# zyhbili/Dual-Space-NeRF

Measured on AMD Instinct MI355X. Metric: rendered rays/sec (64 samples/ray), 512x512 frame, higher is better.
Workload: dtype split-f16x3 (3 x v_mfma_f32_32x32x16_f16 on hi/lo fp16 operand halves, f32 accumulate: f32-equivalent accuracy - parity bars of the tests: 1e-4 absolute on RGB / acc / weights against the reference; sigma 1e-4 absolute where |sigma| <= 100 and 4e-6 RELATIVE to max|sigma| above (this checkpoint: |sig

## Files before the change

dual-space-nerf_amd/csrc/dsn_common.h:

```cpp
#pragma once
#include <hip/hip_runtime.h>
#include <stddef.h>
#include <stdint.h>

#define DSN_WAVE 64
#define DSN_NUM_PARAMS_INTERNAL 33

struct DsnFaceRec {
    float m0[3];
    float d00;
    float v10[3];
    float d01;
    float v20[3];
    float d11;
    float n[3];
    float inv;
};

#ifndef DSN_LIGHT_RECORD_FLOATS
#define DSN_LIGHT_RECORD_FLOATS 12
#endif
struct DsnLightEdit {
    float has_light, light_shift[3], has_rot, rot[4] , rot_center[2], pad;
};
static_assert(sizeof(DsnLightEdit) == 4 * DSN_LIGHT_RECORD_FLOATS, "DsnLightEdit is one light record");
__device__ __forceinline__ void dsn_light_edit(const DsnLightEdit& e, float (&xw)[3]) {
    if (e.has_rot != 0.0f) {
        const float ax = xw[0] - e.rot_center[0], ay = xw[1] - e.rot_center[1];
        const float nx = (ax * e.rot[0] + ay * e.rot[2]) + e.rot_center[0];
        const float ny = (ax * e.rot[1] + ay * e.rot[3]) + e.rot_center[1];
        xw[0] = nx; xw[1] = ny;
    }
    if (e.has_light != 0.0f) { xw[0] += e.light_shift[0]; xw[1] += e.light_shift[1]; xw[2] += e.light_shift[2]; }
}

struct DsnFrameState {
    float pose_feat[16];
    float code[8];
    DsnLightEdit light;
    float pad[28];
    float bias0[256];
};
static_assert(offsetof(DsnFrameState, bias0) == 256 && sizeof(DsnFrameState) == 1280, "DsnFrameState layout");

__host__ __device__ inline size_t dsn_align256(size_t x) { return (x + 255) & ~(size_t)255; }
#include "dsn_nn.h"

struct DsnSceneView {
    int V, F;
    float* canon;
    int32_t* faces;
    float* xyz;
    float4* cent_world;
    float4* cent_canon;
    DsnFaceRec* face_world;
    DsnFaceRec* face_canon;
    DsnFrameState* frame;
    DsnNNView nn_world;
    DsnNNView nn_canon;
};

__host__ __device__ inline DsnSceneView dsn_scene_view(void* base, int V, int F) {
    DsnSceneView s;
    char* p = (char*)base;
    s.V = V; s.F = F;
    p += 256;
    s.frame = (DsnFrameState*)p;    p += dsn_align256(sizeof(DsnFrameState));
    s.canon = (float*)p;            p += dsn_align256(sizeof(float) * 3 * (size_t)V);
    s.faces = (int32_t*)p;          p += dsn_align256(sizeof(int32_t) * 3 * (size_t)F);
    s.xyz = (float*)p;              p += dsn_align256(sizeof(float) * 3 * (size_t)V);
    s.cent_world = (float4*)p;      p += dsn_align256(sizeof(float4) * (size_t)F);
    s.cent_canon = (float4*)p;      p += dsn_align256(sizeof(float4) * (size_t)F);
    s.face_world = (DsnFaceRec*)p;  p += dsn_align256(sizeof(DsnFaceRec) * (size_t)F);
    s.face_canon = (DsnFaceRec*)p;  p += dsn_align256(sizeof(DsnFaceRec) * (size_t)F);
    s.nn_world = dsn_nn_view(p, F);
    s.nn_canon = dsn_nn_view(p, F);
    return s;
}
__host__ __device__ inline size_t dsn_pose_state_size() { return 256 + dsn_align256(sizeof(DsnFrameState)); }
__host__ __device__ inline size_t dsn_scene_size(int V, int F) {
    return 256 + 2 * dsn_align256(sizeof(float) * 3 * (size_t)V) + dsn_align256(sizeof(int32_t) * 3 * (size_t)F) +
           2 * dsn_align256(sizeof(float4) * (size_t)F) + 2 * dsn_align256(sizeof(DsnFaceRec) * (size_t)F) +
           dsn_align256(sizeof(DsnFrameState)) + 2 * dsn_nn_bytes(F);
}

__device__ __forceinline__ float dsn_sum3(float a, float b, float c) { return (a + b) + c; }
__device__ __forceinline__ float dsn_dot3(const float* a, const float* b) {
    return dsn_sum3(a[0] * b[0], a[1] * b[1], a[2] * b[2]);
}
__device__ __forceinline__ float dsn_norm3(const float* a) {
    return sqrtf(fmaf(a[2], a[2], fmaf(a[1], a[1], a[0] * a[0])));
}
__device__ __forceinline__ void dsn_cross3(const float* a, const float* b, float* o) {
    o[0] = fmaf(a[1], b[2], -(a[2] * b[1]));
    o[1] = fmaf(a[2], b[0], -(a[0] * b[2]));
    o[2] = fmaf(a[0], b[1], -(a[1] * b[0]));
}
__device__ __forceinline__ float dsn_div(float a, float b) { return __fdiv_rn(a, b); }

__device__ __forceinline__ void dsn_sincos(float x, float& s, float& c) {
    const float kf = rintf(x * 0.636619772367581343f);
    float r = fmaf(kf, -1.57079637050628662109375f, x);
    r = fmaf(kf, 4.37113900018624283e-8f, r);
    const float z = r * r;
    float ps = fmaf(z, -1.9515295891e-4f, 8.3321608736e-3f);
    ps = fmaf(z, ps, -1.6666654611e-1f);
    const float sr = fmaf(r * z, ps, r);
    float pc = fmaf(z, 2.443315711809948e-5f, -1.388731625493765e-3f);
    pc = fmaf(z, pc, 4.166664568298827e-2f);
    const float cr = fmaf(z * z, pc, fmaf(z, -0.5f, 1.0f));
    const int q = (int)kf;
    const float a = (q & 1) ? cr : sr;
    const float b = (q & 1) ? sr : cr;
    s = (q & 2) ? -a : a;
    c = ((q + 1) & 2) ? -b : b;
}
// ... 122 lines not shown
```

dual-space-nerf_amd/csrc/dsn_field16.hip:

```cpp
#include "dsn_common.h"
#include "dsn_kernels.h"

typedef float f32x16 __attribute__((ext_vector_type(16)));
typedef _Float16 half8 __attribute__((ext_vector_type(8)));
#define MFMA16(a, b, c) __builtin_amdgcn_mfma_f32_32x32x16_f16((a), (b), (c), 0, 0, 0)

#if !defined(DSN_EXPERIMENTS) && (defined(F16_ABL) || defined(F16_SABL) || defined(F16_TIMING) || defined(F16_TRAIN_ABL))
#error "F16_ABL / F16_SABL / F16_TIMING are experiment switches (wrong results / debug counters): build with -DDSN_EXPERIMENTS"
#endif
#ifndef F16_SINCOS_OCML
#define F16_SINCOS_OCML 0
#endif
#ifndef F16_FENCE
#define F16_FENCE 0
#endif
#ifndef F16_SGB
#define F16_SGB 1
#endif
#ifndef F16_SGB_VALU
#define F16_SGB_VALU 2
#endif
#ifndef F16_SGB_DS
#define F16_SGB_DS 1
#endif
#ifndef F16_MIX
#define F16_MIX 1
#endif
#ifndef F16_PIPE_LATE
#define F16_PIPE_LATE 1
#endif
#ifndef F16_ABL
#define F16_ABL 0
#endif
#ifndef F16_NEXT_POINT
#define F16_NEXT_POINT 1
#endif
#ifndef F16_DMA_SPREAD
#define F16_DMA_SPREAD 1
#endif
#ifndef F16_BIAS_AHEAD
#define F16_BIAS_AHEAD 1
#endif
#ifndef F16_TIMING
#define F16_TIMING 0
#endif
#ifndef F16_PREFETCH
#define F16_PREFETCH 1
#endif

#define F16_THREADS 256
#if defined(DSN_EXPERIMENTS) && defined(F16_TRAIN_ABL) && (F16_TRAIN_ABL & 32)
#define F16_ST_M(m) (1024 * (m))
#else
#define F16_ST_M(m) (32 * (m))
#endif
#define F16_CHUNK 8
#define F16_RING_SLOTS (2 * F16_CHUNK)
#define F16_NCHUNK (DSN_STREAM_BLOCKS / F16_CHUNK)
#define F16_RANGE 65000.0f
#define F16_RANGE_SCALED 32768.0f
#define F16_GSCALE 0.015625f
#define F16_GUNSCALE 64.0f

#if F16_TIMING
__device__ unsigned long long g_f16_timing[16];
#define F16_STAMP(i) do { if (MODE == F16_FWD) { asm volatile("s_waitcnt vmcnt(0) lgkmcnt(0)" ::: "memory"); tstamp[i] = __builtin_readcyclecounter(); rstamp[i] = wall_clock64(); } } while (0)
extern "C" __attribute__((visibility("default"))) int dsn_debug_timing(unsigned long long* out16, int reset) {
    if (out16 && hipMemcpyFromSymbol(out16, HIP_SYMBOL(g_f16_timing), sizeof(unsigned long long) * 16) != hipSuccess) return 1;
    if (reset) { unsigned long long z[16] = {0}; if (hipMemcpyToSymbol(HIP_SYMBOL(g_f16_timing), z, sizeof(z)) != hipSuccess) return 1; }
    return 0;
}
#else
#define F16_STAMP(i) do { } while (0)
#endif
struct W16 {
    const char* g;
    char* ring;
    unsigned ring_off;
    int wave;
    int nchunk = F16_NCHUNK;
    bool spread = F16_DMA_SPREAD != 0;
    half8 h0, l0, h1, l1;
};

#ifndef F16_POS_OFFS
#define F16_POS_OFFS 0
#endif
__device__ __forceinline__ void w16_stage(const W16& w, int c) {
    const char* src = w.g + (size_t)c * 32768;
    const unsigned dst = w.ring_off + (c & 1) * 32768 + w.wave * 8192 + 4096;
#if F16_POS_OFFS
// ... 124 lines not shown
#endif
            __builtin_amdgcn_sched_group_barrier(0x002, F16_SGB_VALU, 0);
        }
        __builtin_amdgcn_sched_barrier(0);
#endif
#if F16_FENCE
        __builtin_amdgcn_sched_barrier(0);
#endif
    }
}

__device__ __forceinline__ f32x16 rows16(const float* __restrict__ v, int m, int half) {
    f32x16 o;
#pragma unroll
    for (int q = 0; q < 4; ++q) {
        const float4 t = *reinterpret_cast<const float4*>(v + 32 * m + 8 * q + 4 * half);
        o[4 * q + 0] = t.x; o[4 * q + 1] = t.y; o[4 * q + 2] = t.z; o[4 * q + 3] = t.w;
    }
    return o;
}
__device__ __forceinline__ f32x16 zero16() {
    f32x16 z;
#pragma unroll
    for (int r = 0; r < 16; ++r) z[r] = 0.0f;
    return z;
}
template <bool SCALED>
__device__ __forceinline__ void split16(const f32x16& v, half8 (&h)[2], half8 (&l)[2]) {
#pragma unroll
    for (int r = 0; r < 16; ++r) {
        const _Float16 hi = (_Float16)v[r];
        const float res = fmaf((float)hi, -1.0f, v[r]);
        h[r >> 3][r & 7] = hi;
        l[r >> 3][r & 7] = SCALED ? (_Float16)(res * DSN_LO_SCALE) : (_Float16)res;
    }
}
#define F16_FWD_SCALE 64.0f
#define F16_FWD_INV 0.015625f
__device__ __forceinline__ f32x16 unscale16(const f32x16& m, const f32x16& c) {
    f32x16 v;
#pragma unroll
    for (int r = 0; r < 16; ++r) v[r] = (m[r] + c[r]) * F16_FWD_INV;
    return v;
}
__device__ __forceinline__ f32x16 fold16(const f32x16& m, const f32x16& c) {
    f32x16 v;
#pragma unroll
    for (int r = 0; r < 16; ++r) v[r] = fmaf(c[r], DSN_LO_INV, m[r]);
    return v;
}
__device__ __forceinline__ uint32_t dsn_push_sign(uint32_t word, float v) {
    return __builtin_amdgcn_alignbit(word, __float_as_uint(v), 31);
}
__device__ __forceinline__ uint32_t dsn_active_word(uint32_t signs) { return ~signs & 0xffffu; }
#ifndef F16_KEEP_ASM
#define F16_KEEP_ASM 1
#endif
__device__ __forceinline__ float dsn_keep_active(float v, uint32_t word, int r) {
#if F16_KEEP_ASM
    uint32_t m;
    asm("v_bfe_i32 %0, %1, %2, 1" : "=v"(m) : "v"(word), "s"(15 - r));
    return __uint_as_float(__float_as_uint(v) & m);
#else
    return __uint_as_float(__float_as_uint(v) & (uint32_t)__builtin_amdgcn_sbfe((int)word, 15 - r, 1));
#endif
}
__device__ __forceinline__ uint32_t relu_bits16(f32x16& a) {
    uint32_t s = 0;
#pragma unroll
    for (int r = 0; r < 16; ++r) {
        s = dsn_push_sign(s, a[r]);
        a[r] = fmaxf(a[r], 0.0f);
    }
    return dsn_active_word(s);
}
__device__ __forceinline__ void mask16(f32x16& a, uint32_t m) {
#pragma unroll
    for (int r = 0; r < 16; ++r) a[r] = dsn_keep_active(a[r], m, r);
}

__device__ __forceinline__ void track16(float& ovf, const f32x16& v) {
#pragma unroll
    for (int r = 0; r < 16; r += 2) asm("v_max3_f32 %0, %0, |%1|, |%2|" : "+v"(ovf) : "v"(v[r]), "v"(v[r + 1]));
}
__device__ __forceinline__ float dsn_nan_flag() { return __uint_as_float(0x7fc00000u); }

#if defined(DSN_EXPERIMENTS) && defined(F16_TRAIN_ABL) && (F16_TRAIN_ABL & 256)
__device__ __forceinline__ void store16_lines_emul(float* st, const float (&o)[16]) {
    const int lane = threadIdx.x & 63;
    const unsigned long long me = (unsigned long long)(uintptr_t)st;
#pragma unroll
    for (int j = 0; j < 4; ++j) {
        const int src = 8 * j + (lane >> 3);
        const unsigned lo = __shfl((unsigned)me, src), hi = __shfl((unsigned)(me >> 32), src);
        float* pj = reinterpret_cast<float*>((uintptr_t)(((unsigned long long)hi << 32) | lo));
        if (pj) *reinterpret_cast<float4*>(pj + 4 * (lane & 7)) = make_float4(o[4 * j], o[4 * j + 1], o[4 * j + 2], o[4 * j + 3]);
    }
}
#endif
template <bool FWD, bool ST = false, bool HEAD = false>
__device__ __forceinline__ void epi_slice(const f32x16& pM, const f32x16& pC, int kb, uint32_t mword, uint32_t& bits,
                                          half8 (&yh)[2], half8 (&yl)[2], float& ovf, float* st = nullptr, float stscale = 1.0f,
                                          const float* wd = nullptr, float* sg = nullptr) {
#if F16_ABL & 16
    {
        asm volatile("" : : "a"(pM[2 * kb]), "a"(pM[2 * kb + 1]), "a"(pC[2 * kb]), "a"(pC[2 * kb + 1]));
        if (kb == 0) { yh[0] = yh[1]; yl[0] = yl[1]; }
        return;
    }
#endif
    float vv[2];
#pragma unroll
    for (int e = 0; e < 2; ++e) {
        const int r = 2 * kb + e;
#if F16_ABL & 32
        asm volatile("" : : "v"(pC[r]));
        float v = FWD ? pM[r] * F16_FWD_INV : pM[r];
#else
        float v = FWD ? (pM[r] + pC[r]) * F16_FWD_INV : fmaf(pC[r], DSN_LO_INV, pM[r]);
#endif
        if (FWD) {
            bits = dsn_push_sign(bits, v);
            v = fmaxf(v, 0.0f);
        } else {
            v = dsn_keep_active(v, mword, r);
        }
        vv[e] = v;
        if (HEAD) *sg = fmaf(wd[8 * (r >> 2) + (r & 3)], v, *sg);
#if !F16_MIX
        const _Float16 hi = (_Float16)v;
        const float res = fmaf((float)hi, -1.0f, v);
        yh[r >> 3][r & 7] = hi;
        yl[r >> 3][r & 7] = FWD ? (_Float16)res : (_Float16)(res * DSN_LO_SCALE);
#endif
    }
#if F16_MIX
    {
        const int r = 2 * kb;
        uint32_t H, L;
        asm("v_cvt_pk_f16_f32 %0, %1, %2" : "=v"(H) : "v"(vv[0]), "v"(vv[1]));
        if (FWD) {
            asm("v_fma_mixlo_f16 %0, %1, -1.0, %2 op_sel_hi:[1,0,0]" : "=v"(L) : "v"(H), "v"(vv[0]));
            asm("v_fma_mixhi_f16 %0, %1, -1.0, %2 op_sel:[1,0,0] op_sel_hi:[1,0,0]" : "+v"(L) : "v"(H), "v"(vv[1]));
        } else {
            const float k = -DSN_LO_SCALE;
            const float s0 = vv[0] * DSN_LO_SCALE, s1 = vv[1] * DSN_LO_SCALE;
            asm("v_fma_mixlo_f16 %0, %1, %2, %3 op_sel_hi:[1,0,0]" : "=v"(L) : "v"(H), "s"(k), "v"(s0));
            asm("v_fma_mixhi_f16 %0, %1, %2, %3 op_sel:[1,0,0] op_sel_hi:[1,0,0]" : "+v"(L) : "v"(H), "s"(k), "v"(s1));
        }
        typedef uint32_t u32x4 __attribute__((ext_vector_type(4)));
        u32x4 th = __builtin_bit_cast(u32x4, yh[r >> 3]), tl = __builtin_bit_cast(u32x4, yl[r >> 3]);
        th[(r & 7) >> 1] = H;
        tl[(r & 7) >> 1] = L;
        yh[r >> 3] = __builtin_bit_cast(half8, th);
        yl[r >> 3] = __builtin_bit_cast(half8, tl);
    }
#endif
    if (FWD) asm("v_max3_f32 %0, %0, %1, %2" : "+v"(ovf) : "v"(vv[0]), "v"(vv[1]));
    else asm("v_max3_f32 %0, %0, |%1|, |%2|" : "+v"(ovf) : "v"(vv[0]), "v"(vv[1]));
#if defined(DSN_EXPERIMENTS) && defined(F16_TRAIN_ABL) && (F16_TRAIN_ABL & 256)
    if (ST && kb == 7) {
        float o[16];
#pragma unroll
        for (int r = 0; r < 16; ++r) {
            float v = FWD ? (pM[r] + pC[r]) * F16_FWD_INV : fmaf(pC[r], DSN_LO_INV, pM[r]);
            v = FWD ? fmaxf(v, 0.0f) : dsn_keep_active(v, mword, r);
// ... 1494 lines not shown
    for (int m = 0; m < 4; ++m) {
        f32x16 acc = rows16(packed + OFF_BLT1, m, half);
#pragma unroll
        for (int kb = 0; kb < 4; ++kb) {
            const float4* bp = reinterpret_cast<const float4*>(packed + OFF_LT1 + (m * 4 + kb) * DSN_BLK) + lane;
            const float4 c0 = bp[0], c1 = bp[64], c2 = bp[128], c3 = bp[192];
            acc = DSN_MFMA(c0.x, h1[kb][0], acc);  acc = DSN_MFMA(c0.y, h1[kb][1], acc);
            acc = DSN_MFMA(c0.z, h1[kb][2], acc);  acc = DSN_MFMA(c0.w, h1[kb][3], acc);
            acc = DSN_MFMA(c1.x, h1[kb][4], acc);  acc = DSN_MFMA(c1.y, h1[kb][5], acc);
            acc = DSN_MFMA(c1.z, h1[kb][6], acc);  acc = DSN_MFMA(c1.w, h1[kb][7], acc);
            acc = DSN_MFMA(c2.x, h1[kb][8], acc);  acc = DSN_MFMA(c2.y, h1[kb][9], acc);
            acc = DSN_MFMA(c2.z, h1[kb][10], acc); acc = DSN_MFMA(c2.w, h1[kb][11], acc);
            acc = DSN_MFMA(c3.x, h1[kb][12], acc); acc = DSN_MFMA(c3.y, h1[kb][13], acc);
            acc = DSN_MFMA(c3.z, h1[kb][14], acc); acc = DSN_MFMA(c3.w, h1[kb][15], acc);
        }
#pragma unroll
        for (int r = 0; r < 16; ++r) acc[r] = acc[r] > 0.0f ? acc[r] : 0.0f;
        h2[m] = acc;
    }
    float part = 0.0f;
#pragma unroll
    for (int m = 0; m < 4; ++m) {
        const f32x16 w = rows16(packed + OFF_WLT2, m, half);
#pragma unroll
        for (int r = 0; r < 16; ++r) part = fmaf(w[r], h2[m][r], part);
    }
    part += __shfl_xor(part, 32);
    return part + packed[OFF_SCAL + 4];
}

#define LIGHT32_THREADS 256
__global__ void __launch_bounds__(LIGHT32_THREADS, 1)
k_light(const float* __restrict__ packed, const DsnFrameState* __restrict__ fs, const float* __restrict__ n_w,
        const float* __restrict__ x_w_pts, const float* __restrict__ ray_o, const float* __restrict__ ray_d,
        const float* __restrict__ z_vals, const float* essence, int64_t N, int S,
        const int32_t* __restrict__ active_list, const int32_t* __restrict__ active_count,
        float* colour) {
    DSN_OWN_SIMD();
    const int lane = threadIdx.x & 63;
    const int wave = __builtin_amdgcn_readfirstlane(threadIdx.x >> 6);
    const int half = lane >> 5;
    const int64_t count = active_list ? (int64_t)(*active_count) : N;
    const int64_t slot0 = ((int64_t)blockIdx.x * 4 + wave) * 32;
    if (slot0 >= count) return;
    int64_t slot = slot0 + (lane & 31);
    const bool valid = slot < count;
    if (!valid) slot = count - 1;
    const int64_t pt = active_list ? (int64_t)active_list[slot] : slot;
    const int64_t ray = pt / S;

    float in9[10];
    in9[0] = n_w[3 * pt]; in9[1] = n_w[3 * pt + 1]; in9[2] = n_w[3 * pt + 2];
    float xw[3];
    const float d[3] = {ray_d[3 * ray], ray_d[3 * ray + 1], ray_d[3 * ray + 2]};
    if (x_w_pts) { xw[0] = x_w_pts[3 * pt]; xw[1] = x_w_pts[3 * pt + 1]; xw[2] = x_w_pts[3 * pt + 2]; }
    else {
        const float z = z_vals[pt];
        xw[0] = ray_o[3 * ray] + d[0] * z; xw[1] = ray_o[3 * ray + 1] + d[1] * z; xw[2] = ray_o[3 * ray + 2] + d[2] * z;
    }
    dsn_light_edit(fs->light, xw);
    in9[3] = xw[0]; in9[4] = xw[1]; in9[5] = xw[2];
    const float vn = dsn_norm3(d);
    in9[6] = dsn_div(d[0], vn); in9[7] = dsn_div(d[1], vn); in9[8] = dsn_div(d[2], vn);
    in9[9] = 0.0f;

    const float o = dsn_light_mlp32(packed, lane, in9);
    const float wgt = (o > 0.0f ? o : expm1f(o)) + 1.0f;
    if (valid && half == 0) {
        colour[3 * pt + 0] = wgt * essence[3 * pt + 0];
        colour[3 * pt + 1] = wgt * essence[3 * pt + 1];
        colour[3 * pt + 2] = wgt * essence[3 * pt + 2];
    }
}

void dsn_launch_light(const float* packed, const DsnFrameState* fs, const float* n_w, const float* x_w,
                      const float* ray_o, const float* ray_d, const float* z_vals, const float* essence, int64_t N,
                      int S, const int32_t* active_list, const int32_t* active_count, float* colour, hipStream_t st) {
    int64_t blocks = (N + 127) / 128;
    if (blocks == 0) return;
    hipLaunchKernelGGL(k_light, dim3((unsigned)blocks), dim3(LIGHT32_THREADS), 0, st, packed, fs, n_w, x_w, ray_o, ray_d,
                       z_vals, essence, N, S, active_list, active_count, colour);
}

__device__ __forceinline__ void light_block0(const char* blkp, int lane, const half8 (&xh)[2], const half8 (&xl)[2], f32x16& aM, f32x16& aC) {
    const half8 h0 = *reinterpret_cast<const half8*>(blkp + lane * 16);
    const half8 l0 = *reinterpret_cast<const half8*>(blkp + 1024 + lane * 16);
    aM = MFMA16(h0, xh[0], aM);
    aC = MFMA16(h0, xl[0], aC);
    aC = MFMA16(l0, xh[0], aC);
}
__device__ __forceinline__ void light_block(const char* __restrict__ blkp, int lane, const half8 (&xh)[2], const half8 (&xl)[2],
                                            f32x16& aM, f32x16& aC, bool second_step) {
    const half8 h0 = *reinterpret_cast<const half8*>(blkp + lane * 16);
    const half8 l0 = *reinterpret_cast<const half8*>(blkp + 1024 + lane * 16);
    aM = MFMA16(h0, xh[0], aM);
    aC = MFMA16(h0, xl[0], aC);
    aC = MFMA16(l0, xh[0], aC);
    if (second_step) {
        const half8 h1 = *reinterpret_cast<const half8*>(blkp + 2048 + lane * 16);
        const half8 l1 = *reinterpret_cast<const half8*>(blkp + 3072 + lane * 16);
        aM = MFMA16(h1, xh[1], aM);
        aC = MFMA16(h1, xl[1], aC);
        aC = MFMA16(l1, xh[1], aC);
    }
}

#define LIGHT_LDS_BYTES (4 * 2048 + 16 * 4096)
__device__ __forceinline__ void light16_stage_weights(const float* __restrict__ packed, char* s_w) {
    const char* g16 = reinterpret_cast<const char*>(packed + OFF16_BASE);
    const uint4* g0 = reinterpret_cast<const uint4*>(g16 + (size_t)(OFF_LT0 / DSN_BLK) * 4096);
    const uint4* g1 = reinterpret_cast<const uint4*>(g16 + (size_t)(OFF_LT1 / DSN_BLK) * 4096);
    uint4* d = reinterpret_cast<uint4*>(s_w);
    for (int i = threadIdx.x; i < 4 * 128; i += 256) d[i] = g0[(i >> 7) * 256 + (i & 127)];
    for (int i = threadIdx.x; i < 16 * 256; i += 256) d[4 * 128 + i] = g1[i];
    __syncthreads();
}
struct LightIn { float nw[3], o[3], d[3], z; };
__device__ __forceinline__ int64_t light16_tile_slot(int64_t t, int wave, int lane, int64_t ntiles, int64_t count, bool& ok) {
    int64_t sl = (t * 4 + wave) * 32 + (lane & 31);
    ok = t < ntiles && sl < count;
    if (!ok) sl = count - 1;
    return sl;
}
__device__ __forceinline__ void light16_fetch(int64_t p, int S, const float* __restrict__ n_w, const float* __restrict__ x_w_pts,
                                              const float* __restrict__ ray_o, const float* __restrict__ ray_d,
                                              const float* __restrict__ z_vals, LightIn& a) {
    const int64_t r = p / S;
    a.nw[0] = n_w[3 * p]; a.nw[1] = n_w[3 * p + 1]; a.nw[2] = n_w[3 * p + 2];
    a.d[0] = ray_d[3 * r]; a.d[1] = ray_d[3 * r + 1]; a.d[2] = ray_d[3 * r + 2];
    if (x_w_pts) { a.o[0] = x_w_pts[3 * p]; a.o[1] = x_w_pts[3 * p + 1]; a.o[2] = x_w_pts[3 * p + 2]; a.z = 0.0f; }
    else { a.o[0] = ray_o[3 * r]; a.o[1] = ray_o[3 * r + 1]; a.o[2] = ray_o[3 * r + 2]; a.z = z_vals[p]; }
}
__device__ __forceinline__ float light16_mlp(const float* __restrict__ packed, const char* s_w, int lane, const float (&in9)[10],
                                             bool valid, int64_t pt, float* __restrict__ tr_hl1, float* __restrict__ tr_hl2,
                                             bool& flagged) {
    const int half = lane >> 5;
    float ovf = packed[DSN_SPLIT_UNSAFE_LIGHT];
    half8 xh[2], xl[2];
    {
        f32x16 v = zero16();
#pragma unroll
        for (int j = 0; j < 5; ++j) v[j] = half ? in9[2 * j + 1] : in9[2 * j];
        track16(ovf, v);
        split16<true>(v, xh, xl);
    }
    half8 h1h[4][2], h1l[4][2];
#pragma unroll
    for (int m = 0; m < 4; ++m) {
        f32x16 aM = rows16(packed + OFF_BLT0, m, half), aC = zero16();
        light_block0(s_w + m * 2048, lane, xh, xl, aM, aC);
        f32x16 v = fold16(aM, aC);
#pragma unroll
        for (int r = 0; r < 16; ++r) v[r] = fmaxf(v[r], 0.0f);
        if (tr_hl1 && valid) store16(tr_hl1 + pt * 128 + 4 * half + 32 * m, v, 1.0f);
        track16(ovf, v);
        split16<true>(v, h1h[m], h1l[m]);
    }
    float part = 0.0f;
#pragma unroll
    for (int m = 0; m < 4; ++m) {
        f32x16 aM = rows16(packed + OFF_BLT1, m, half), aC = zero16();
#pragma unroll
        for (int kb = 0; kb < 4; ++kb)
            light_block(s_w + 4 * 2048 + (m * 4 + kb) * 4096, lane, h1h[kb], h1l[kb], aM, aC, true);
        f32x16 v = fold16(aM, aC);
        const f32x16 w2 = rows16(packed + OFF_WLT2, m, half);
#pragma unroll
        for (int r = 0; r < 16; ++r) { v[r] = fmaxf(v[r], 0.0f); part = fmaf(w2[r], v[r], part); }
        if (tr_hl2 && valid) store16(tr_hl2 + pt * 128 + 4 * half + 32 * m, v, 1.0f);
    }
    part += __shfl_xor(part, 32);
    float o = part + packed[OFF_SCAL + 4];
    flagged = !(fmaxf(ovf, __shfl_xor(ovf, 32)) < F16_RANGE_SCALED);
    if (__ballot(flagged)) {
        const float e = dsn_light_mlp32(packed, lane, in9);
        if (flagged) o = e;
    }
    return o;
}
__device__ __forceinline__ float light16_weight(float o) { return (o > 0.0f ? o : expm1f(o)) + 1.0f; }

template <bool FACTOR>
__global__ void __launch_bounds__(256, 1)
k_light16(const float* __restrict__ packed, const DsnFrameState* __restrict__ fs, const float* __restrict__ n_w,
          const float* __restrict__ x_w_pts, const float* __restrict__ ray_o, const float* __restrict__ ray_d,
          const float* __restrict__ z_vals, const float* essence, int64_t N, int S,
          const int32_t* __restrict__ active_list, const int32_t* __restrict__ active_count,
          float* colour, float* __restrict__ tr_hl1, float* __restrict__ tr_hl2, float* __restrict__ tr_pre,
          int32_t* __restrict__ range_count, float* __restrict__ factor) {
    __shared__ __attribute__((aligned(16))) char s_w[LIGHT_LDS_BYTES];
#ifndef F16_SHARE_SIMD
    DSN_OWN_SIMD();
#endif
    const int lane = threadIdx.x & 63;
    const int wave = __builtin_amdgcn_readfirstlane(threadIdx.x >> 6);
    const int half = lane >> 5;
    const int64_t count = active_list ? (int64_t)(*active_count) : N;
    const int64_t ntiles = (count + 127) / 128;
    if ((int64_t)blockIdx.x >= ntiles) return;
    light16_stage_weights(packed, s_w);
    auto tile_pt = [&](int64_t t, bool& ok) -> int64_t {
        const int64_t sl = light16_tile_slot(t, wave, lane, ntiles, count, ok);
        return active_list ? (int64_t)active_list[sl] : sl;
    };
    bool valid_c, valid_n, valid_nn;
    int64_t pt_c = tile_pt(blockIdx.x, valid_c);
    LightIn in_c, in_n;
    light16_fetch(pt_c, S, n_w, x_w_pts, ray_o, ray_d, z_vals, in_c);
    int64_t pt_n = tile_pt((int64_t)blockIdx.x + gridDim.x, valid_n);
  for (int64_t tile = blockIdx.x; tile < ntiles; tile += gridDim.x) {
    const int64_t slot0 = (tile * 4 + wave) * 32;
    const bool valid = valid_c;
    const int64_t pt = pt_c;
    const LightIn cur = in_c;
    light16_fetch(pt_n, S, n_w, x_w_pts, ray_o, ray_d, z_vals, in_n);
    const int64_t pt_nn = tile_pt(tile + 2 * (int64_t)gridDim.x, valid_nn);
    pt_c = pt_n; valid_c = valid_n; in_c = in_n;
    pt_n = pt_nn; valid_n = valid_nn;
    if (slot0 >= count) continue;
    const float ess[3] = {essence[3 * pt], essence[3 * pt + 1], essence[3 * pt + 2]};

    float in9[10];
    in9[0] = cur.nw[0]; in9[1] = cur.nw[1]; in9[2] = cur.nw[2];
    float xw[3];
    const float d[3] = {cur.d[0], cur.d[1], cur.d[2]};
    if (x_w_pts) { xw[0] = cur.o[0]; xw[1] = cur.o[1]; xw[2] = cur.o[2]; }
    else {
        const float z = cur.z;
        xw[0] = cur.o[0] + d[0] * z; xw[1] = cur.o[1] + d[1] * z; xw[2] = cur.o[2] + d[2] * z;
    }
    dsn_light_edit(fs->light, xw);
    in9[3] = xw[0]; in9[4] = xw[1]; in9[5] = xw[2];
    const float vn = dsn_norm3(d);
    in9[6] = dsn_div(d[0], vn); in9[7] = dsn_div(d[1], vn); in9[8] = dsn_div(d[2], vn);
    in9[9] = 0.0f;

    bool flagged;
    const float o = light16_mlp(packed, s_w, lane, in9, valid, pt, tr_hl1, tr_hl2, flagged);
    if (flagged && range_count && valid && half == 0) atomicAdd(range_count, 1);
    const float wgt = light16_weight(o);
    if (tr_pre && valid && half == 0) tr_pre[pt] = o;
    if (valid && half == 0) {
        colour[3 * pt + 0] = wgt * ess[0];
        colour[3 * pt + 1] = wgt * ess[1];
        colour[3 * pt + 2] = wgt * ess[2];
        if (FACTOR) factor[pt] = wgt;
    }
  }
}

void dsn_launch_light16(const float* packed, const DsnFrameState* fs, const float* n_w, const float* x_w,
                        const float* ray_o, const float* ray_d, const float* z_vals, const float* essence, int64_t N,
                        int S, const int32_t* active_list, const int32_t* active_count, float* colour, hipStream_t st,
                        float* tr_hl1, float* tr_hl2, float* tr_pre, int32_t* range_count, float* factor) {
    int64_t blocks = (N + 127) / 128;
    if (blocks == 0) return;
    const dim3 grid((unsigned)std::min<int64_t>(blocks, (int64_t)dsn_cu_count()));
    if (factor)
        hipLaunchKernelGGL(k_light16<true>, grid, dim3(256), 0, st, packed, fs, n_w, x_w, ray_o, ray_d, z_vals, essence, N, S, active_list,
                           active_count, colour, tr_hl1, tr_hl2, tr_pre, range_count, factor);
    else
        hipLaunchKernelGGL(k_light16<false>, grid, dim3(256), 0, st, packed, fs, n_w, x_w, ray_o, ray_d, z_vals, essence, N, S, active_list,
                           active_count, colour, tr_hl1, tr_hl2, tr_pre, range_count, factor);
}

template <bool FACTOR>
__global__ void __launch_bounds__(256, 1)
k_light16_multi(const float* __restrict__ packed, const DsnLightEdit* __restrict__ lights, int G, const float* __restrict__ n_w,
                const float* __restrict__ ray_o, const float* __restrict__ ray_d, const float* __restrict__ z_vals,
                const float* __restrict__ essence, int S, const int32_t* __restrict__ list, const int32_t* __restrict__ list_count,
                float* __restrict__ colours, float* __restrict__ factors) {
    __shared__ __attribute__((aligned(16))) char s_w[LIGHT_LDS_BYTES];
#ifndef F16_SHARE_SIMD
    DSN_OWN_SIMD();
#endif
    const int lane = threadIdx.x & 63;
    const int wave = __builtin_amdgcn_readfirstlane(threadIdx.x >> 6);
    const int half = lane >> 5;
    const int64_t count = *list_count;
    const int64_t ntiles = (count + 127) / 128;
    if ((int64_t)blockIdx.x >= ntiles) return;
    light16_stage_weights(packed, s_w);
    auto tile_pt = [&](int64_t t, bool& ok) -> int64_t { return (int64_t)list[light16_tile_slot(t, wave, lane, ntiles, count, ok)]; };
    bool valid_c, valid_n, valid_nn;
    int64_t pt_c = tile_pt(blockIdx.x, valid_c);
    LightIn in_c, in_n;
    light16_fetch(pt_c, S, n_w, nullptr, ray_o, ray_d, z_vals, in_c);
    int64_t pt_n = tile_pt((int64_t)blockIdx.x + gridDim.x, valid_n);
  for (int64_t tile = blockIdx.x; tile < ntiles; tile += gridDim.x) {
    const int64_t slot0 = (tile * 4 + wave) * 32;
    const int64_t slot = slot0 + (lane & 31);
    const bool valid = valid_c;
    const int64_t pt = pt_c;
    const LightIn cur = in_c;
    light16_fetch(pt_n, S, n_w, nullptr, ray_o, ray_d, z_vals, in_n);
    const int64_t pt_nn = tile_pt(tile + 2 * (int64_t)gridDim.x, valid_nn);
    pt_c = pt_n; valid_c = valid_n; in_c = in_n;
    pt_n = pt_nn; valid_n = valid_nn;
    if (slot0 >= count) continue;
    const float ess[3] = {essence[3 * pt], essence[3 * pt + 1], essence[3 * pt + 2]};
    const float d[3] = {cur.d[0], cur.d[1], cur.d[2]};
    float xw0[3];
    {
        const float z = cur.z;
        xw0[0] = cur.o[0] + d[0] * z; xw0[1] = cur.o[1] + d[1] * z; xw0[2] = cur.o[2] + d[2] * z;
    }
    const float vn = dsn_norm3(d);
    const float vd[3] = {dsn_div(d[0], vn), dsn_div(d[1], vn), dsn_div(d[2], vn)};
    for (int g = 0; g < G; ++g) {
        asm volatile("" ::: "memory");
        float in9[10];
        in9[0] = cur.nw[0]; in9[1] = cur.nw[1]; in9[2] = cur.nw[2];
        float xw[3] = {xw0[0], xw0[1], xw0[2]};
        dsn_light_edit(lights[g], xw);
        in9[3] = xw[0]; in9[4] = xw[1]; in9[5] = xw[2];
        in9[6] = vd[0]; in9[7] = vd[1]; in9[8] = vd[2];
        in9[9] = 0.0f;
        bool flagged;
        const float wgt = light16_weight(light16_mlp(packed, s_w, lane, in9, valid, pt, nullptr, nullptr, flagged));
        if (valid && half == 0) {
            float* c = colours + ((int64_t)g * count + slot) * 3;
            c[0] = wgt * ess[0];
            c[1] = wgt * ess[1];
            c[2] = wgt * ess[2];
            if (FACTOR) factors[(int64_t)g * count + slot] = wgt;
        }
    }
  }
}

void dsn_launch_light16_multi(const float* packed, const DsnLightEdit* lights, int G, const float* n_w, const float* ray_o, const float* ray_d,
                              const float* z_vals, const float* essence, int64_t max_count, int S, const int32_t* list,
                              const int32_t* list_count, float* colours, hipStream_t st, float* factors) {
    const int64_t blocks = (max_count + 127) / 128;
    if (blocks == 0 || G < 1) return;
    const dim3 grid((unsigned)std::min<int64_t>(blocks, (int64_t)dsn_cu_count()));
    if (factors)
        hipLaunchKernelGGL(k_light16_multi<true>, grid, dim3(256), 0, st, packed, lights, G, n_w, ray_o, ray_d, z_vals, essence, S, list,
                           list_count, colours, factors);
    else
        hipLaunchKernelGGL(k_light16_multi<false>, grid, dim3(256), 0, st, packed, lights, G, n_w, ray_o, ray_d, z_vals, essence, S, list,
                           list_count, colours, factors);
}
```

Baseline: 30.59 million.

## Software-pipeline light MLP layers across consecutive points with interleaved MFMA schedule

Restructures the fp16 split light MLP so that the first-layer MFMAs and epilogue for the next tile or light are interleaved, slot by slot under sched_barrier, with the second-layer MFMAs of the current one. It also prefetches weight fragments from LDS ahead of use, stages biases and output weights into LDS, and makes the light edit branchless. The goal is to hide VALU epilogue and LDS latency behind MFMA issue. The cost is much higher register pressure and complex manual scheduling, which can lower occupancy or cause spills.

```diff
diff --git a/dual-space-nerf_amd/csrc/dsn_common.h b/dual-space-nerf_amd/csrc/dsn_common.h
--- a/dual-space-nerf_amd/csrc/dsn_common.h
+++ b/dual-space-nerf_amd/csrc/dsn_common.h
@@ -25,13 +25,13 @@
 };
 static_assert(sizeof(DsnLightEdit) == 4 * DSN_LIGHT_RECORD_FLOATS, "DsnLightEdit is one light record");
 __device__ __forceinline__ void dsn_light_edit(const DsnLightEdit& e, float (&xw)[3]) {
-    if (e.has_rot != 0.0f) {
-        const float ax = xw[0] - e.rot_center[0], ay = xw[1] - e.rot_center[1];
-        const float nx = (ax * e.rot[0] + ay * e.rot[2]) + e.rot_center[0];
-        const float ny = (ax * e.rot[1] + ay * e.rot[3]) + e.rot_center[1];
-        xw[0] = nx; xw[1] = ny;
-    }
-    if (e.has_light != 0.0f) { xw[0] += e.light_shift[0]; xw[1] += e.light_shift[1]; xw[2] += e.light_shift[2]; }
+    const bool rot = e.has_rot != 0.0f, shift = e.has_light != 0.0f;
+    const float ax = xw[0] - e.rot_center[0], ay = xw[1] - e.rot_center[1];
+    const float nx = (ax * e.rot[0] + ay * e.rot[2]) + e.rot_center[0];
+    const float ny = (ax * e.rot[1] + ay * e.rot[3]) + e.rot_center[1];
+    xw[0] = rot ? nx : xw[0]; xw[1] = rot ? ny : xw[1];
+    const float sx = xw[0] + e.light_shift[0], sy = xw[1] + e.light_shift[1], sz = xw[2] + e.light_shift[2];
+    xw[0] = shift ? sx : xw[0]; xw[1] = shift ? sy : xw[1]; xw[2] = shift ? sz : xw[2];
 }
 
 struct DsnFrameState {
diff --git a/dual-space-nerf_amd/csrc/dsn_field16.hip b/dual-space-nerf_amd/csrc/dsn_field16.hip
--- a/dual-space-nerf_amd/csrc/dsn_field16.hip
+++ b/dual-space-nerf_amd/csrc/dsn_field16.hip
@@ -5,8 +5,8 @@
 typedef _Float16 half8 __attribute__((ext_vector_type(8)));
 #define MFMA16(a, b, c) __builtin_amdgcn_mfma_f32_32x32x16_f16((a), (b), (c), 0, 0, 0)
 
-#if !defined(DSN_EXPERIMENTS) && (defined(F16_ABL) || defined(F16_SABL) || defined(F16_TIMING) || defined(F16_TRAIN_ABL))
-#error "F16_ABL / F16_SABL / F16_TIMING are experiment switches (wrong results / debug counters): build with -DDSN_EXPERIMENTS"
+#if !defined(DSN_EXPERIMENTS) && (defined(F16_ABL) || defined(F16_SABL) || defined(F16_TIMING) || defined(F16_TRAIN_ABL) || defined(LIGHT_ABL))
+#error "F16_ABL / F16_SABL / F16_TIMING / LIGHT_ABL are experiment switches (wrong results / debug counters): build with -DDSN_EXPERIMENTS"
 #endif
 #ifndef F16_SINCOS_OCML
 #define F16_SINCOS_OCML 0
@@ -297,6 +297,16 @@
 __device__ __forceinline__ void track16(float& ovf, const f32x16& v) {
 #pragma unroll
     for (int r = 0; r < 16; r += 2) asm("v_max3_f32 %0, %0, |%1|, |%2|" : "+v"(ovf) : "v"(v[r]), "v"(v[r + 1]));
+}
+__device__ __forceinline__ void track16(float& ovf, const f32x16& v, int r) {
+    asm("v_max3_f32 %0, %0, |%1|, |%2|" : "+v"(ovf) : "v"(v[r]), "v"(v[r + 1]));
+}
+template <bool SCALED>
+__device__ __forceinline__ void split16(const f32x16& v, half8 (&h)[2], half8 (&l)[2], int r) {
+    const _Float16 hi = (_Float16)v[r];
+    const float res = fmaf((float)hi, -1.0f, v[r]);
+    h[r >> 3][r & 7] = hi;
+    l[r >> 3][r & 7] = SCALED ? (_Float16)(res * DSN_LO_SCALE) : (_Float16)res;
 }
 __device__ __forceinline__ float dsn_nan_flag() { return __uint_as_float(0x7fc00000u); }
 
@@ -1957,30 +1967,71 @@
                        z_vals, essence, N, S, active_list, active_count, colour);
 }
 
-__device__ __forceinline__ void light_block0(const char* blkp, int lane, const half8 (&xh)[2], const half8 (&xl)[2], f32x16& aM, f32x16& aC) {
-    const half8 h0 = *reinterpret_cast<const half8*>(blkp + lane * 16);
-    const half8 l0 = *reinterpret_cast<const half8*>(blkp + 1024 + lane * 16);
-    aM = MFMA16(h0, xh[0], aM);
-    aC = MFMA16(h0, xl[0], aC);
-    aC = MFMA16(l0, xh[0], aC);
-}
-__device__ __forceinline__ void light_block(const char* __restrict__ blkp, int lane, const half8 (&xh)[2], const half8 (&xl)[2],
-                                            f32x16& aM, f32x16& aC, bool second_step) {
-    const half8 h0 = *reinterpret_cast<const half8*>(blkp + lane * 16);
-    const half8 l0 = *reinterpret_cast<const half8*>(blkp + 1024 + lane * 16);
-    aM = MFMA16(h0, xh[0], aM);
-    aC = MFMA16(h0, xl[0], aC);
-    aC = MFMA16(l0, xh[0], aC);
-    if (second_step) {
-        const half8 h1 = *reinterpret_cast<const half8*>(blkp + 2048 + lane * 16);
-        const half8 l1 = *reinterpret_cast<const half8*>(blkp + 3072 + lane * 16);
-        aM = MFMA16(h1, xh[1], aM);
-        aC = MFMA16(h1, xl[1], aC);
-        aC = MFMA16(l1, xh[1], aC);
-    }
-}
-
-#define LIGHT_LDS_BYTES (4 * 2048 + 16 * 4096)
+#ifndef LIGHT_SGB_VALU
+#define LIGHT_SGB_VALU 5
+#endif
+#ifndef LIGHT_ABL
+#define LIGHT_ABL 0
+#endif
+#if LIGHT_ABL & 2
+__device__ __forceinline__ f32x16 light_no_mfma(const half8& a, const half8& b, const f32x16& c) { asm volatile("" : : "v"(a), "v"(b)); return c; }
+#define LMFMA16(a, b, c) light_no_mfma((a), (b), (c))
+#else
+#define LMFMA16(a, b, c) MFMA16((a), (b), (c))
+#endif
+struct LightW { half8 h0, l0, h1, l1; };
+__device__ __forceinline__ void light_wread(const char* blkp, int lane, LightW& w, int step) {
+    half8& h = step ? w.h1 : w.h0;
+    half8& l = step ? w.l1 : w.l0;
+#if LIGHT_ABL & 4
+    const half8 z = {0, 0, 0, 0, 0, 0, 0, 0};
+    h = z; l = z;
+    asm volatile("" : "+v"(h), "+v"(l) : "v"(blkp));
+    return;
+#endif
+    h = *reinterpret_cast<const half8*>(blkp + 2048 * step + lane * 16);
+    l = *reinterpret_cast<const half8*>(blkp + 2048 * step + 1024 + lane * 16);
+}
+__device__ __forceinline__ void light_first_mfma(int i, const LightW& wa, const LightW& wb, const half8& xh, const half8& xl, f32x16& aMa,
+                                                 f32x16& aCa, f32x16& aMb, f32x16& aCb) {
+    if (i == 0) aCa = LMFMA16(wa.h0, xl, aCa);
+    if (i == 1) aCb = LMFMA16(wb.h0, xl, aCb);
+    if (i == 2) aMa = LMFMA16(wa.h0, xh, aMa);
+    if (i == 3) aCa = LMFMA16(wa.l0, xh, aCa);
+    if (i == 4) aCb = LMFMA16(wb.l0, xh, aCb);
+    if (i == 5) aMb = LMFMA16(wb.h0, xh, aMb);
+}
+#define LIGHT_SLOT(i) do { hook(i); __builtin_amdgcn_sched_barrier(0); } while (0)
+template <class Hook>
+__device__ __forceinline__ void light_pair(const LightW& wa, const LightW& wb, const half8 (&xh)[2], const half8 (&xl)[2], f32x16& aMa,
+                                           f32x16& aCa, f32x16& aMb, f32x16& aCb, Hook&& hook) {
+    aCa = LMFMA16(wa.h0, xl[0], aCa); LIGHT_SLOT(0);
+    aCb = LMFMA16(wb.h0, xl[0], aCb); LIGHT_SLOT(1);
+    aMa = LMFMA16(wa.h0, xh[0], aMa); LIGHT_SLOT(2);
+    aCa = LMFMA16(wa.l0, xh[0], aCa); LIGHT_SLOT(3);
+    aCb = LMFMA16(wb.l0, xh[0], aCb); LIGHT_SLOT(4);
+    aMb = LMFMA16(wb.h0, xh[0], aMb); LIGHT_SLOT(5);
+    aCa = LMFMA16(wa.h1, xl[1], aCa); LIGHT_SLOT(6);
+    aCb = LMFMA16(wb.h1, xl[1], aCb); LIGHT_SLOT(7);
+    aMa = LMFMA16(wa.h1, xh[1], aMa); LIGHT_SLOT(8);
+    aCa = LMFMA16(wa.l1, xh[1], aCa); LIGHT_SLOT(9);
+    aCb = LMFMA16(wb.l1, xh[1], aCb); LIGHT_SLOT(10);
+    aMb = LMFMA16(wb.h1, xh[1], aMb); LIGHT_SLOT(11);
+}
+__device__ __forceinline__ void light_epi2(const f32x16& aM, const f32x16& aC, const f32x16& w2, int r, float& part, f32x16& keep) {
+#if LIGHT_ABL & 1
+    {
+        asm volatile("" : : "v"(aM[r]), "v"(aC[r]));
+        return;
+    }
+#endif
+    const float v = fmaxf(fmaf(aC[r], DSN_LO_INV, aM[r]), 0.0f);
+    keep[r] = v;
+    part = fmaf(w2[r], v, part);
+}
+
+#define LIGHT_W_BYTES (4 * 2048 + 16 * 4096)
+#define LIGHT_LDS_BYTES (LIGHT_W_BYTES + 3 * 128 * 4)
 __device__ __forceinline__ void light16_stage_weights(const float* __restrict__ packed, char* s_w) {
     const char* g16 = reinterpret_cast<const char*>(packed + OFF16_BASE);
     const uint4* g0 = reinterpret_cast<const uint4*>(g16 + (size_t)(OFF_LT0 / DSN_BLK) * 4096);
@@ -1988,6 +2039,11 @@
     uint4* d = reinterpret_cast<uint4*>(s_w);
     for (int i = threadIdx.x; i < 4 * 128; i += 256) d[i] = g0[(i >> 7) * 256 + (i & 127)];
     for (int i = threadIdx.x; i < 16 * 256; i += 256) d[4 * 128 + i] = g1[i];
+    if (threadIdx.x < 96) {
+        const int row = threadIdx.x >> 5, i = threadIdx.x & 31;
+        const float* src = packed + (row == 0 ? OFF_BLT0 : row == 1 ? OFF_BLT1 : OFF_WLT2);
+        reinterpret_cast<float4*>(s_w + LIGHT_W_BYTES)[threadIdx.x] = reinterpret_cast<const float4*>(src)[i];
+    }
     __syncthreads();
 }
 struct LightIn { float nw[3], o[3], d[3], z; };
@@ -2000,55 +2056,163 @@
 __device__ __forceinline__ void light16_fetch(int64_t p, int S, const float* __restrict__ n_w, const float* __restrict__ x_w_pts,
                                               const float* __restrict__ ray_o, const float* __restrict__ ray_d,
                                               const float* __restrict__ z_vals, LightIn& a) {
+#if LIGHT_ABL & 8
+    a.nw[0] = 0.6f; a.nw[1] = 0.0f; a.nw[2] = 0.8f; a.d[0] = 0.0f; a.d[1] = 0.0f; a.d[2] = 1.0f; a.o[0] = (float)(p & 7); a.o[1] = 0.5f; a.o[2] = 0.25f; a.z = 1.0f;
+    return;
+#endif
     const int64_t r = p / S;
     a.nw[0] = n_w[3 * p]; a.nw[1] = n_w[3 * p + 1]; a.nw[2] = n_w[3 * p + 2];
     a.d[0] = ray_d[3 * r]; a.d[1] = ray_d[3 * r + 1]; a.d[2] = ray_d[3 * r + 2];
     if (x_w_pts) { a.o[0] = x_w_pts[3 * p]; a.o[1] = x_w_pts[3 * p + 1]; a.o[2] = x_w_pts[3 * p + 2]; a.z = 0.0f; }
     else { a.o[0] = ray_o[3 * r]; a.o[1] = ray_o[3 * r + 1]; a.o[2] = ray_o[3 * r + 2]; a.z = z_vals[p]; }
 }
-__device__ __forceinline__ float light16_mlp(const float* __restrict__ packed, const char* s_w, int lane, const float (&in9)[10],
-                                             bool valid, int64_t pt, float* __restrict__ tr_hl1, float* __restrict__ tr_hl2,
-                                             bool& flagged) {
+struct LightOp { half8 xh, xl; float ovf; };
+__device__ __forceinline__ void light16_in9(int i, const LightIn& a, bool world_pts, const DsnLightEdit& e, float (&in9)[10], float& vn) {
+    if (i == 0 || i < 0) {
+        in9[0] = a.nw[0]; in9[1] = a.nw[1]; in9[2] = a.nw[2];
+        float xw[3];
+#pragma unroll
+        for (int c = 0; c < 3; ++c) { const float q = a.o[c] + a.d[c] * a.z; xw[c] = world_pts ? a.o[c] : q; }
+        dsn_light_edit(e, xw);
+        in9[3] = xw[0]; in9[4] = xw[1]; in9[5] = xw[2];
+        in9[9] = 0.0f;
+    }
+    if (i == 1 || i < 0) vn = dsn_norm3(a.d);
+    if (i == 3 || i < 0) in9[6] = dsn_div(a.d[0], vn);
+    if (i == 4 || i < 0) in9[7] = dsn_div(a.d[1], vn);
+    if (i == 6 || i < 0) in9[8] = dsn_div(a.d[2], vn);
+}
+struct LightH { half8 h[4][2], l[4][2]; float ovf; };
+__device__ __forceinline__ void light_epi1(const f32x16& aM, const f32x16& aC, int r, half8 (&h)[2], half8 (&l)[2], float& ovf, f32x16& keep);
+__device__ __forceinline__ void light16_input_a(const float (&in9)[10], int half, float ovf0, f32x16& v, float& ovf);
+__device__ __forceinline__ void light16_input_b(const f32x16& v, float ovf, LightOp& op);
+__device__ __forceinline__ void light16_input(const float (&in9)[10], int half, float ovf0, LightOp& op);
+template <bool TRAIN, class Next>
+__device__ __forceinline__ float light16_mlp(const char* s_w, int lane, const LightH& H, float bias_out, float* st2,
+                                                bool& flagged, Next&& next, const LightOp& in_n, float* st1_n, LightH& Hn) {
     const int half = lane >> 5;
-    float ovf = packed[DSN_SPLIT_UNSAFE_LIGHT];
-    half8 xh[2], xl[2];
+    const float* rows = reinterpret_cast<const float*>(s_w + LIGHT_W_BYTES);
+    const char* s_w2 = s_w + 4 * 2048;
+    f32x16 bM[4], bC[4], aM[4], aC[4], keep, keep2[2], w2[2];
+    LightW wc[2], wn[2], w1[2];
+    float part = 0.0f, ovf_n = 0.0f;
+#pragma unroll
+    for (int q = 0; q < 4; ++q) light_wread(s_w2 + ((q >> 1) * 4 + 0) * 4096, lane, wc[q >> 1], q & 1);
+#pragma unroll
+    for (int P = 0; P < 2; ++P) {
+        const int a = 2 * P, b = 2 * P + 1;
+        aM[a] = rows16(rows + 128, a, half); aC[a] = zero16();
+        aM[b] = rows16(rows + 128, b, half); aC[b] = zero16();
+#pragma unroll
+        for (int kb = 0; kb < 4; ++kb) {
+            const int r = 4 * P + kb;
+            light_pair(wc[0], wc[1], H.h[kb], H.l[kb], aM[a], aC[a], aM[b], aC[b], [&](int i) {
+                if (i % 3 == 2 && r < 7) {
+                    const int q = i / 3, na = kb < 3 ? a : 2, nkb = kb < 3 ? kb + 1 : 0;
+                    light_wread(s_w2 + ((na + (q >> 1)) * 4 + nkb) * 4096, lane, wn[q >> 1], q & 1);
+                }
+                const int e = r == 2 ? i : r == 3 ? 12 + i : r == 5 ? (i < 8 ? 24 + i : 24 + i) : r == 6 ? 36 + i : r == 7 ? 48 + i : -1;
+                if (r == 0) {
+                    next(i);
+                    if (i == 11) ovf_n = in_n.ovf;
+                } else if (r == 1) {
+                    if (i == 0) { bM[0] = rows16(rows, 0, half); bC[0] = zero16(); bM[1] = rows16(rows, 1, half); bC[1] = zero16(); }
+                    if (i == 1) { light_wread(s_w, lane, w1[0], 0); light_wread(s_w + 2048, lane, w1[1], 0); }
+                    if (i >= 3 && i < 9) light_first_mfma(i - 3, w1[0], w1[1], in_n.xh, in_n.xl, bM[0], bC[0], bM[1], bC[1]);
+                } else if (r == 4) {
+                    if (i == 0) { w2[0] = rows16(rows + 256, 0, half); w2[1] = rows16(rows + 256, 1, half); }
+                    if (i >= 1) {
+#pragma unroll
+                        for (int q = 3 * (i - 1); q < 3 * i && q < 32; ++q) light_epi2(aM[q >> 4], aC[q >> 4], w2[q >> 4], q & 15, part, keep2[q >> 4]);
+                    }
+                    if (TRAIN && i == 11) { store16(st2, keep2[0], 1.0f); store16(st2 ? st2 + 32 : nullptr, keep2[1], 1.0f); }
+                } else {
+                    if (r == 5) {
+                        if (i == 0) { bM[2] = rows16(rows, 2, half); bC[2] = zero16(); bM[3] = rows16(rows, 3, half); bC[3] = zero16(); }
+                        if (i == 1) { light_wread(s_w + 2 * 2048, lane, w1[0], 0); light_wread(s_w + 3 * 2048, lane, w1[1], 0); }
+                        if (i >= 2 && i < 8) light_first_mfma(i - 2, w1[0], w1[1], in_n.xh, in_n.xl, bM[2], bC[2], bM[3], bC[3]);
+                    }
+                    light_epi1(bM[e >> 4], bC[e >> 4], e & 15, Hn.h[e >> 4], Hn.l[e >> 4], ovf_n, keep);
+                    if (TRAIN && (e & 15) == 15) store16(st1_n ? st1_n + 32 * (e >> 4) : nullptr, keep, 1.0f);
+                }
+            });
+            if (r < 7) { wc[0] = wn[0]; wc[1] = wn[1]; }
+        }
+    }
+#pragma unroll
+    for (int r = 12; r < 16; ++r) light_epi1(bM[3], bC[3], r, Hn.h[3], Hn.l[3], ovf_n, keep);
+    if (TRAIN) store16(st1_n ? st1_n + 96 : nullptr, keep, 1.0f);
+#pragma unroll
+    for (int m = 2; m < 4; ++m) {
+        const f32x16 w = rows16(rows + 256, m, half);
+#pragma unroll
+        for (int r = 0; r < 16; ++r) light_epi2(aM[m], aC[m], w, r, part, keep2[0]);
+        if (TRAIN) store16(st2 ? st2 + 32 * m : nullptr, keep2[0], 1.0f);
+    }
+    Hn.ovf = ovf_n;
+    part += __shfl_xor(part, 32);
+    flagged = !(fmaxf(H.ovf, __shfl_xor(H.ovf, 32)) < F16_RANGE_SCALED);
+    return part + bias_out;
+}
+__device__ __forceinline__ void light_epi1(const f32x16& aM, const f32x16& aC, int r, half8 (&h)[2], half8 (&l)[2], float& ovf, f32x16& keep) {
+#if LIGHT_ABL & 1
     {
-        f32x16 v = zero16();
-#pragma unroll
-        for (int j = 0; j < 5; ++j) v[j] = half ? in9[2 * j + 1] : in9[2 * j];
-        track16(ovf, v);
-        split16<true>(v, xh, xl);
-    }
-    half8 h1h[4][2], h1l[4][2];
+        asm volatile("" : : "v"(aM[r]), "v"(aC[r]));
+        h[r >> 3][r & 7] = (_Float16)0.0f; l[r >> 3][r & 7] = (_Float16)0.0f;
+        return;
+    }
+#endif
+    const float v = fmaxf(fmaf(aC[r], DSN_LO_INV, aM[r]), 0.0f);
+    keep[r] = v;
+    if (r & 1) track16(ovf, keep, r - 1);
+    split16<true>(keep, h, l, r);
+}
+__device__ __forceinline__ void light16_input_a(const float (&in9)[10], int half, float ovf0, f32x16& v, float& ovf) {
+    v = zero16();
+#pragma unroll
+    for (int j = 0; j < 5; ++j) v[j] = half ? in9[2 * j + 1] : in9[2 * j];
+    ovf = ovf0;
+    track16(ovf, v);
+}
+__device__ __forceinline__ void light16_input_b(const f32x16& v, float ovf, LightOp& op) {
+    half8 h[2], l[2];
+    split16<true>(v, h, l);
+    op.xh = h[0]; op.xl = l[0]; op.ovf = ovf;
+}
+__device__ __forceinline__ void light16_input(const float (&in9)[10], int half, float ovf0, LightOp& op) {
+    f32x16 v;
+    float ovf;
+    light16_input_a(in9, half, ovf0, v, ovf);
+    light16_input_b(v, ovf, op);
+}
+template <bool TRAIN>
+__device__ __forceinline__ void light16_first(const char* s_w, int lane, const LightOp& in, float* st1, LightH& H) {
+    const int half = lane >> 5;
+    const float* rows = reinterpret_cast<const float*>(s_w + LIGHT_W_BYTES);
+    f32x16 bM[4], bC[4], keep;
+    LightW w1[4];
+    float ovf = in.ovf;
+#pragma unroll
+    for (int m = 0; m < 4; ++m) light_wread(s_w + m * 2048, lane, w1[m], 0);
+#pragma unroll
+    for (int m = 0; m < 4; ++m) { bM[m] = rows16(rows, m, half); bC[m] = zero16(); }
+#pragma unroll
+    for (int i = 0; i < 6; ++i) light_first_mfma(i, w1[0], w1[1], in.xh, in.xl, bM[0], bC[0], bM[1], bC[1]);
+#pragma unroll
+    for (int i = 0; i < 6; ++i) light_first_mfma(i, w1[2], w1[3], in.xh, in.xl, bM[2], bC[2], bM[3], bC[3]);
 #pragma unroll
     for (int m = 0; m < 4; ++m) {
-        f32x16 aM = rows16(packed + OFF_BLT0, m, half), aC = zero16();
-        light_block0(s_w + m * 2048, lane, xh, xl, aM, aC);
-        f32x16 v = fold16(aM, aC);
-#pragma unroll
-        for (int r = 0; r < 16; ++r) v[r] = fmaxf(v[r], 0.0f);
-        if (tr_hl1 && valid) store16(tr_hl1 + pt * 128 + 4 * half + 32 * m, v, 1.0f);
-        track16(ovf, v);
-        split16<true>(v, h1h[m], h1l[m]);
-    }
-    float part = 0.0f;
-#pragma unroll
-    for (int m = 0; m < 4; ++m) {
-        f32x16 aM = rows16(packed + OFF_BLT1, m, half), aC = zero16();
-#pragma unroll
-        for (int kb = 0; kb < 4; ++kb)
-            light_block(s_w + 4 * 2048 + (m * 4 + kb) * 4096, lane, h1h[kb], h1l[kb], aM, aC, true);
-        f32x16 v = fold16(aM, aC);
-        const f32x16 w2 = rows16(packed + OFF_WLT2, m, half);
-#pragma unroll
-        for (int r = 0; r < 16; ++r) { v[r] = fmaxf(v[r], 0.0f); part = fmaf(w2[r], v[r], part); }
-        if (tr_hl2 && valid) store16(tr_hl2 + pt * 128 + 4 * half + 32 * m, v, 1.0f);
-    }
-    part += __shfl_xor(part, 32);
-    float o = part + packed[OFF_SCAL + 4];
-    flagged = !(fmaxf(ovf, __shfl_xor(ovf, 32)) < F16_RANGE_SCALED);
+#pragma unroll
+        for (int r = 0; r < 16; ++r) light_epi1(bM[m], bC[m], r, H.h[m], H.l[m], ovf, keep);
+        if (TRAIN) store16(st1 ? st1 + 32 * m : nullptr, keep, 1.0f);
+    }
+    H.ovf = ovf;
+}
+__device__ __forceinline__ float light16_exact(const float* __restrict__ packed, int lane, const float (&in9)[10], bool flagged, float o) {
     if (__ballot(flagged)) {
-        const float e = dsn_light_mlp32(packed, lane, in9);
+        const float* pk = packed;
+        asm volatile("" : "+s"(pk));
+        const float e = dsn_light_mlp32(pk, lane, in9);
         if (flagged) o = e;
     }
     return o;
@@ -2074,44 +2238,63 @@
     const int64_t ntiles = (count + 127) / 128;
     if ((int64_t)blockIdx.x >= ntiles) return;
     light16_stage_weights(packed, s_w);
+    const float ovf0 = packed[DSN_SPLIT_UNSAFE_LIGHT], bias_out = packed[OFF_SCAL + 4];
+    const bool world_pts = x_w_pts != nullptr, train = tr_hl1 != nullptr || tr_hl2 != nullptr;
     auto tile_pt = [&](int64_t t, bool& ok) -> int64_t {
         const int64_t sl = light16_tile_slot(t, wave, lane, ntiles, count, ok);
         return active_list ? (int64_t)active_list[sl] : sl;
     };
     bool valid_c, valid_n, valid_nn;
     int64_t pt_c = tile_pt(blockIdx.x, valid_c);
-    LightIn in_c, in_n;
-    light16_fetch(pt_c, S, n_w, x_w_pts, ray_o, ray_d, z_vals, in_c);
+    LightIn in_n;
+    light16_fetch(pt_c, S, n_w, x_w_pts, ray_o, ray_d, z_vals, in_n);
     int64_t pt_n = tile_pt((int64_t)blockIdx.x + gridDim.x, valid_n);
-  for (int64_t tile = blockIdx.x; tile < ntiles; tile += gridDim.x) {
+    float in9[2][10];
+    LightOp op;
+    LightH H[2];
+    {
+        float vn;
+        light16_in9(-1, in_n, world_pts, fs->light, in9[0], vn);
+    }
+    light16_input(in9[0], half, ovf0, op);
+    {
+        float* st1 = (tr_hl1 && valid_c) ? tr_hl1 + pt_c * 128 + 4 * half : nullptr;
+        if (train) light16_first<true>(s_w, lane, op, st1, H[0]);
+        else light16_first<false>(s_w, lane, op, nullptr, H[0]);
+    }
+  for (int64_t tile0 = blockIdx.x; tile0 < ntiles; tile0 += 2 * (int64_t)gridDim.x) {
+#pragma unroll
+   for (int u = 0; u < 2; ++u) {
+    const int64_t tile = tile0 + u * (int64_t)gridDim.x;
+    if (tile >= ntiles) break;
     const int64_t slot0 = (tile * 4 + wave) * 32;
     const bool valid = valid_c;
     const int64_t pt = pt_c;
-    const LightIn cur = in_c;
     light16_fetch(pt_n, S, n_w, x_w_pts, ray_o, ray_d, z_vals, in_n);
     const int64_t pt_nn = tile_pt(tile + 2 * (int64_t)gridDim.x, valid_nn);
-    pt_c = pt_n; valid_c = valid_n; in_c = in_n;
+    pt_c = pt_n; valid_c = valid_n;
     pt_n = pt_nn; valid_n = valid_nn;
-    if (slot0 >= count) continue;
+    if (slot0 >= count) break;
     const float ess[3] = {essence[3 * pt], essence[3 * pt + 1], essence[3 * pt + 2]};
 
-    float in9[10];
-    in9[0] = cur.nw[0]; in9[1] = cur.nw[1]; in9[2] = cur.nw[2];
-    float xw[3];
-    const float d[3] = {cur.d[0], cur.d[1], cur.d[2]};
-    if (x_w_pts) { xw[0] = cur.o[0]; xw[1] = cur.o[1]; xw[2] = cur.o[2]; }
-    else {
-        const float z = cur.z;
-        xw[0] = cur.o[0] + d[0] * z; xw[1] = cur.o[1] + d[1] * z; xw[2] = cur.o[2] + d[2] * z;
-    }
-    dsn_light_edit(fs->light, xw);
-    in9[3] = xw[0]; in9[4] = xw[1]; in9[5] = xw[2];
-    const float vn = dsn_norm3(d);
-    in9[6] = dsn_div(d[0], vn); in9[7] = dsn_div(d[1], vn); in9[8] = dsn_div(d[2], vn);
-    in9[9] = 0.0f;
-
+    LightOp op_n;
+    float vn_n, ovf_n;
+    f32x16 v_n;
+    auto next = [&](int i) {
+        light16_in9(i, in_n, world_pts, fs->light, in9[u ^ 1], vn_n);
+        if (i == 7) light16_input_a(in9[u ^ 1], half, ovf0, v_n, ovf_n);
+        if (i == 9) light16_input_b(v_n, ovf_n, op_n);
+    };
     bool flagged;
-    const float o = light16_mlp(packed, s_w, lane, in9, valid, pt, tr_hl1, tr_hl2, flagged);
+    float o;
+    if (train) {
+        float* st1_n = (tr_hl1 && valid_c) ? tr_hl1 + pt_c * 128 + 4 * half : nullptr;
+        float* st2 = (tr_hl2 && valid) ? tr_hl2 + pt * 128 + 4 * half : nullptr;
+        o = light16_mlp<true>(s_w, lane, H[u], bias_out, st2, flagged, next, op_n, st1_n, H[u ^ 1]);
+    } else {
+        o = light16_mlp<false>(s_w, lane, H[u], bias_out, nullptr, flagged, next, op_n, nullptr, H[u ^ 1]);
+    }
+    o = light16_exact(packed, lane, in9[u], flagged, o);
     if (flagged && range_count && valid && half == 0) atomicAdd(range_count, 1);
     const float wgt = light16_weight(o);
     if (tr_pre && valid && half == 0) tr_pre[pt] = o;
@@ -2121,6 +2304,7 @@
         colour[3 * pt + 2] = wgt * ess[2];
         if (FACTOR) factor[pt] = wgt;
     }
+   }
   }
 }
 
@@ -2156,6 +2340,7 @@
     const int64_t ntiles = (count + 127) / 128;
     if ((int64_t)blockIdx.x >= ntiles) return;
     light16_stage_weights(packed, s_w);
+    const float ovf0 = packed[DSN_SPLIT_UNSAFE_LIGHT], bias_out = packed[OFF_SCAL + 4];
     auto tile_pt = [&](int64_t t, bool& ok) -> int64_t { return (int64_t)list[light16_tile_slot(t, wave, lane, ntiles, count, ok)]; };
     bool valid_c, valid_n, valid_nn;
     int64_t pt_c = tile_pt(blockIdx.x, valid_c);
@@ -2182,17 +2367,37 @@
     }
     const float vn = dsn_norm3(d);
     const float vd[3] = {dsn_div(d[0], vn), dsn_div(d[1], vn), dsn_div(d[2], vn)};
-    for (int g = 0; g < G; ++g) {
-        asm volatile("" ::: "memory");
-        float in9[10];
-        in9[0] = cur.nw[0]; in9[1] = cur.nw[1]; in9[2] = cur.nw[2];
-        float xw[3] = {xw0[0], xw0[1], xw0[2]};
-        dsn_light_edit(lights[g], xw);
-        in9[3] = xw[0]; in9[4] = xw[1]; in9[5] = xw[2];
-        in9[6] = vd[0]; in9[7] = vd[1]; in9[8] = vd[2];
-        in9[9] = 0.0f;
+    float ovf_n;
+    f32x16 v_n;
+    auto input_of = [&](int i, int g, float (&in9)[10], LightOp& op) {
+        if (i == 0 || i < 0) {
+            in9[0] = cur.nw[0]; in9[1] = cur.nw[1]; in9[2] = cur.nw[2];
+            float xw[3] = {xw0[0], xw0[1], xw0[2]};
+            dsn_light_edit(lights[g], xw);
+            in9[3] = xw[0]; in9[4] = xw[1]; in9[5] = xw[2];
+            in9[6] = vd[0]; in9[7] = vd[1]; in9[8] = vd[2];
+            in9[9] = 0.0f;
+        }
+        if (i == 3 || i < 0) light16_input_a(in9, half, ovf0, v_n, ovf_n);
+        if (i == 6 || i < 0) light16_input_b(v_n, ovf_n, op);
+    };
+    float in9[2][10];
+    LightOp op;
+    LightH H[2];
+    input_of(-1, 0, in9[0], op);
+    light16_first<false>(s_w, lane, op, nullptr, H[0]);
+    for (int g0 = 0; g0 < G; g0 += 2) {
+#pragma unroll
+      for (int u = 0; u < 2; ++u) {
+        const int g = g0 + u;
+        if (g >= G) break;
+        const int gn = g + 1 < G ? g + 1 : g;
+        LightOp op_n;
         bool flagged;
-        const float wgt = light16_weight(light16_mlp(packed, s_w, lane, in9, valid, pt, nullptr, nullptr, flagged));
+        float o = light16_mlp<false>(s_w, lane, H[u], bias_out, nullptr, flagged, [&](int i) { input_of(i, gn, in9[u ^ 1], op_n); }, op_n,
+                                        nullptr, H[u ^ 1]);
+        o = light16_exact(packed, lane, in9[u], flagged, o);
+        const float wgt = light16_weight(o);
         if (valid && half == 0) {
             float* c = colours + ((int64_t)g * count + slot) * 3;
             c[0] = wgt * ess[0];
@@ -2200,6 +2405,7 @@
             c[2] = wgt * ess[2];
             if (FACTOR) factors[(int64_t)g * count + slot] = wgt;
         }
+      }
     }
   }
 }
```

New measurement: 30.43 million. No clear change (-0.5%).
